# LemonATsu/DANBO-pytorch

Measured on AMD Instinct MI355X. Metric: ray-samples/sec at 512x512x64 samples, higher is better.
Workload: dtype f32 (fp16x2-split MFMA products, fp32 accumulate); 1 GPU; H36M danbo_base network, 512x512 rays x (48 coarse + 16 importance) samples, 1 pose / 1 camera per rank, cylinder near/far, exact in-volume culling; rays=262144, samples_per_ray=64, parallelism=rays-dp1

## Files before the change

### danbo-pytorch_amd/core/_hip.py

```python
import ctypes
import os
import re
from ctypes import c_char_p, c_float, c_int, c_void_p
from types import SimpleNamespace

import torch

_HERE = os.path.dirname(os.path.abspath(__file__))
LIB_PATH = os.environ.get("DANBO_HIP_LIB") or os.path.join(os.path.dirname(_HERE), "libdanbo_hip.so")

P = c_void_p
I = c_int
F = c_float


class HeaderError(ValueError):
    """include/danbo_hip.h left the subset of C that parse_header reads"""


_SCALARS = {"int": c_int, "long": ctypes.c_long, "long long": ctypes.c_longlong, "size_t": ctypes.c_size_t, "float": c_float,
            **{f"{u}int{n}_t": getattr(ctypes, f"c_{u}int{n}") for u in ("", "u") for n in (8, 16, 32, 64)}}
_TAIL = r"((?:\*\s*(?:const\b\s*)?)*)(\w+)\s*(?:\[\s*(\w*)\s*\])?$"
_DECL = re.compile(r"(?:const\s+)?(long\s+long|\w+)\b\s*" + _TAIL)
_MORE = re.compile(_TAIL)
# ... 139 lines not shown

def _header_path():
    env = os.environ.get("DANBO_HIP_HEADER")
    tried = [env] if env else [os.path.join(os.path.dirname(LIB_PATH), "danbo_hip.h"),
                               os.path.join(os.path.dirname(os.path.dirname(_HERE)), "include", "danbo_hip.h")]
    for p in tried:
        if os.path.exists(p):
            return p
    raise RuntimeError("danbo_hip.h not found (the ctypes binding is derived from it): tried " + ", ".join(tried)
                       + "; set DANBO_HIP_HEADER or put the header beside the library")


HEADER_PATH = _header_path()
with open(HEADER_PATH) as _f:
    _functions, _structs, _constants = parse_header(_f.read())
SIGNATURES = {name: argtypes for name, (_, argtypes) in _functions.items()}
RESTYPES = {name: restype for name, (restype, _) in _functions.items()}
STRUCTS = {name: type(name, (ctypes.Structure,), {"_fields_": fields, "__doc__": f"struct {name} of include/danbo_hip.h"})
           for name, fields in _structs.items()}
globals().update(STRUCTS)
C = SimpleNamespace(**_constants)
MAX_ROW_SPANS = C.DANBO_MAX_ROW_SPANS
ANERF_MAX_D = C.DANBO_ANERF_MAX_D

TRAIN_TENSORS = (
    ["graph_net.layers.0.lin.weight", "graph_net.layers.0.adj_w", "graph_net.layers.0.bias", "graph_net.layers.1.lin.weight",
     "graph_net.layers.1.adj_w", "graph_net.layers.1.bias", "graph_net.layers.2.weight", "graph_net.layers.2.bias",
     "graph_net.layers.3.weight", "graph_net.layers.3.bias", "graph_net.axis_scale",
     "prob_linears.layers.0.lin.weight", "prob_linears.layers.0.adj_w", "prob_linears.layers.0.bias", "prob_linears.layers.1.weight",
     "prob_linears.layers.1.bias", "prob_linears.layers.2.weight", "prob_linears.layers.2.bias"]
# ... 6 lines not shown
            "framecodes.codes.weight": C.DANBO_T_CODES}
if len(TRAIN_TENSORS) != N_TRAIN_TENSORS or any(TRAIN_TENSORS.index(k) != i for k, i in _anchors.items()):
    raise HeaderError(f"TRAIN_TENSORS does not line up with enum DanboTrainTensor of {HEADER_PATH}")

_lib = None


def lib():
    global _lib
    if _lib is None:
        if not os.path.exists(LIB_PATH):
            raise RuntimeError(
                f"{LIB_PATH} not found: build it with `make -C danbo-pytorch_amd/csrc` "
                "(or __graft_entry__.build()).  There is no CPU / PyTorch fallback.")
        l = ctypes.CDLL(LIB_PATH)
        for name, argtypes in SIGNATURES.items():
            fn = getattr(l, name)
            fn.argtypes = argtypes
            fn.restype = RESTYPES[name]
        if l.danbo_abi_version() != C.DANBO_ABI_VERSION:
            raise RuntimeError(f"{LIB_PATH} has ABI version {l.danbo_abi_version()}, {HEADER_PATH} declares {C.DANBO_ABI_VERSION}: "
                               "the library is stale, rebuild it with `make -C danbo-pytorch_amd/csrc`")
        _lib = l
    return _lib


def ptr(t):
    return None if t is None else c_void_p(t.data_ptr())


def stream():
    return c_void_p(torch.cuda.current_stream().cuda_stream)


# ... 12 lines not shown
```

### danbo-pytorch_amd/core/hip_ops.py

```python
import ctypes

import torch

from . import _hip
from ._hip import call as _call, ptr as _p, stream as _stream

J = _hip.C.DANBO_J
VOL = _hip.C.DANBO_VOL
FEAT = _hip.C.DANBO_FEAT
RAY_FLAT_VMAX = _hip.C.DANBO_RAY_FLAT_VMAX
H_STRIDE = _hip.C.DANBO_H_STRIDE
MLP_PACKED_FLOATS = _hip.C.DANBO_MLP_PACKED_FLOATS
ASSIGN16_PACKED_BYTES = _hip.C.DANBO_ASSIGN16_PACKED_BYTES
MLP16_PACKED_BYTES = _hip.C.DANBO_MLP16_PACKED_BYTES
ANERF_ENC_FLOATS = _hip.C.DANBO_ANERF_ENC_FLOATS
LINEAR16_ENC_K = _hip.C.DANBO_LINEAR16_ENC_K
TRUNK_PACKED_BYTES = _hip.C.DANBO_TRUNK_PACKED_BYTES
TRUNK_PE_WIDTH = _hip.C.DANBO_TRUNK_PE_WIDTH
VIEW_W = 128


def _f32(t, name):
    if t is None:
        return None
# ... 78 lines not shown


def bone_cull(geo, compact=True, cnt=None):
    bits = torch.empty(geo.M, device=geo.device, dtype=torch.int32)
    lst = None
    if compact:
        lst = torch.empty(geo.M, device=geo.device, dtype=torch.int32)
        if cnt is None:
            cnt = torch.zeros(1, device=geo.device, dtype=torch.int32)
        assert cnt.dtype == torch.int32 and cnt.numel() == 1 and cnt.is_contiguous()
    else:
        cnt = None
    rm = tuple(geo.ray_mask) if geo.ray_mask is not None else (None, None, None)
    flat = rm[3] if len(rm) > 3 else None
    _call("danbo_bone_cull", *geo.head(), _p(rm[0]), _p(rm[1]), _p(rm[2]), _p(flat), _p(bits), _p(lst), _p(cnt), _stream())
    return bits, lst, cnt


def ray_bone_mask(rays_o, rays_d, skts, align, axis_scale, t_lo, t_hi, want_flat=False):
    rays_o, rays_d, skts = _f32(rays_o, "rays_o"), _f32(rays_d, "rays_d"), _f32(skts, "skts")
    t_lo, t_hi = _f32(t_lo, "t_lo").reshape(-1), _f32(t_hi, "t_hi").reshape(-1)
    R, G = rays_o.shape[0], skts.shape[0]
    assert t_lo.shape[0] == R and t_hi.shape[0] == R
    mask = torch.empty(R, device=rays_o.device, dtype=torch.int32)
    flat = torch.empty(R, device=rays_o.device, dtype=torch.int32) if want_flat else None
    _call("danbo_ray_bone_mask", _p(rays_o), _p(rays_d), _p(t_lo), _p(t_hi), R, G, _p(skts), _p(_f32(align, "align")),
          _p(_f32(axis_scale, "axis_scale")), _p(mask), _p(flat), _stream())
    return (mask, t_lo, t_hi, flat) if want_flat else (mask, t_lo, t_hi)


# ... 626 lines not shown
```

### danbo-pytorch_amd/core/render_engine.py

```python
import ctypes

import torch

from . import _hip
from . import hip_ops as ops


class RenderEngine:
    fuse_resample = False

    def _key(self):
        return tuple((k, v.data_ptr(), v._version) for k, v in sorted(self.p.items()))

    def _sampling(self, N_samples, N_importance):
        cfg = self.cfg
        return (N_samples or cfg["N_samples"], N_importance or cfg["N_importance"], cfg["density_scale"],
                ops.density_act(cfg.get("density_act")))

    @staticmethod
    def frame_result(out, out0):
        return dict(rgb_map=out["rgb_map"], disp_map=out["disp_map"], acc_map=out["acc_map"], alpha=out["alpha"],
                    T_i=out["weights"], rgb0=out0["rgb_map"], disp0=out0["disp_map"], acc0=out0["acc_map"],
                    alpha0=out0["alpha"])

# ... 161 lines not shown
        self.refresh()
        return ops.pose_volumes(bones, self.gw, self.cfg["multires_graph"])

    def view_constants(self, rays_d, skts, cam_idx, ray_list=None, ray_count=None):
        self.refresh()
        cfg = self.cfg
        ray_mode = {"world": 0, "root_local": 1}[cfg["ray_tr_type"]]
        normalise = 1 if cfg["view_type"] == "relray" else 0
        return ops.view_consts(rays_d, skts, ray_mode, normalise, cfg["multires_views"], self.framecodes,
                               self.mean_code, cam_idx, self.wrt,
                               self.views_b16 if self.mlp_mode == "f16split" else self.views_b, self.rgb_w,
                               self.rgb_b, self.empty_consts, {16: 1, 32: 2}[self.mlp_form] if self.mlp_mode == "f16split" else 0,
                               self.code_table, ray_list, ray_count)

    def forward_samples(self, rays_o, rays_d, skts, bones, cam_idx=None, z=None, pts=None, dense=False,
                        want_confd=False, volumes=None, view=None, fill=True, ray_mask=None, count=None):
        self.refresh()
        geo = ops.Geometry(rays_o, rays_d, skts, self.align, self.axis_scale, z=z, pts=pts, ray_mask=ray_mask)
        vols = self.volumes(bones) if volumes is None else volumes
        cview, raw_empty = self.view_constants(geo.rays_d, geo.skts, cam_idx) if view is None else view
        S = geo.S
        bits, lst, cnt = ops.bone_cull(geo, compact=not dense, cnt=count)
        if lst is not None and self.mlp_mode == "f16split" and self.group_rows:
            ops.group_rows(bits, lst, cnt)
        if self.mlp_mode == "f16split":
            h, confd = ops.gather_assign_blend16(geo, vols, bits, self.aw, self.assign16, lst, cnt, geo.M, want_confd)
        else:
            h, confd = ops.gather_assign_blend(geo, vols, bits, self.aw, lst, cnt, geo.M, want_confd)
        raw = ops.fill_raw(raw_empty, S) if fill or dense else torch.empty(geo.R, S, 4, device=raw_empty.device)
        if self.profile is not None:
            e0, e1 = torch.cuda.Event(enable_timing=True), torch.cuda.Event(enable_timing=True)
            e0.record()
        self._mlp(h, S, cview, raw, lst, cnt, geo.M)
        if self.profile is not None:
            e1.record()
            self.profile.setdefault("k_pe_mlp", []).append((e0, e1, cnt if cnt is not None else geo.M))
        extras = dict(valid_bits=bits, list=lst, count=cnt, confd_rows=confd, h_rows=h, volumes=vols)
# ... 75 lines not shown
        self.refresh()
        near, far = ops.near_far_cylinder(rays_o, rays_d, cyls, near0, far0, chunk)
        if self.cfg["use_volume_near_far"]:
            ops.near_far_boxes(rays_o, rays_d, skts, self.align, self.axis_scale, near, far)
        return near, far

    def render(self, rays_o, rays_d, skts, bones, cyls, cam_idx=None, N_samples=None, N_importance=None,
               chunk=4096, near_far=None, dense=False, keep=False):
        S, Sf, B, act = self._sampling(N_samples, N_importance)
        self.refresh()
        fused = S <= 64 and Sf <= 64
        lazy = not dense and not keep
        flat_mode = (lazy and (fused or (S <= 256 and Sf <= 64)) and self.skip_flat_rays and self.flat_rays_ok
                     and act[0] == "relu")
        near, far = self.near_far(rays_o, rays_d, cyls, skts, 0.0, 1.0, chunk) if near_far is None else near_far
        z = ops.coarse_samples(near, far, S)
        ray_mask = None if dense else ops.ray_bone_mask(rays_o, rays_d, skts, self.align, self.axis_scale, near, far,
                                                        want_flat=flat_mode)
        counts = torch.zeros(3, device=rays_o.device, dtype=torch.int32)
        flat = None
        vols = self.volumes(bones)
        if flat_mode:
            flat = ops.flat_rays(ray_mask[1], ray_mask[3], S, Sf, want_weights=not fused, cnt=counts[2:3])
            view = self.view_constants(rays_d, skts, cam_idx, flat["ray_list"], flat["ray_count"])
        else:
            view = self.view_constants(rays_d, skts, cam_idx)
        if ray_mask is not None:
            ray_mask = ray_mask[:3]
        raw, ex = self.forward_samples(rays_o, rays_d, skts, bones, cam_idx, z=z, dense=dense, volumes=vols, view=view,
                                       fill=not lazy, ray_mask=ray_mask, count=counts[0:1])
        if fused:
            out0, z_all, z_fine, order = ops.composite_importance(
                raw, z, rays_d, Sf, B, bits=ex["valid_bits"] if lazy else None, raw_empty=view[1] if lazy else None,
                want_weights=keep, flat=flat, act=act)
        else:
            out0 = ops.composite(raw, z, rays_d, B, bits=ex["valid_bits"] if lazy else None, raw_empty=view[1] if lazy else None,
                                 flat=flat, act=act)
            z_all, z_fine, order = ops.importance_samples(z, out0["weights"], Sf, flat=flat)
        raw_f, ex_f = self.forward_samples(rays_o, rays_d, skts, bones, cam_idx, z=z_fine, dense=dense,
                                           volumes=vols, view=view, fill=not lazy,
                                           ray_mask=ray_mask, count=counts[1:2])
        out = ops.composite_merged(raw, raw_f, order, z_all, rays_d, B, bits_a=ex["valid_bits"] if lazy else None,
                                   bits_b=ex_f["valid_bits"] if lazy else None, raw_empty=view[1] if lazy else None,
                                   want_raw=keep, flat=flat, act=act)
        ret = self.frame_result(out, out0)
        if keep:
            ret.update(near=near, far=far, z_coarse=z, raw_coarse=raw, weights_coarse=out0["weights"], z_fine=z_fine,
                       z_sorted=z_all, sorted_idxs=order, raw_fine=raw_f, raw_sorted=out.get("raw_sorted"),
                       count_coarse=ex["count"], count_fine=ex_f["count"], valid_bits=ex["valid_bits"])
        return ret

    def _network_pass(self, rays_o, rays_d, skts, bones, cam_idx, z, bounds, dense, lazy, tag):
        mask = None if dense else ops.ray_bone_mask(rays_o, rays_d, skts, self.align, self.axis_scale, *bounds)
        view = self.view_constants(rays_d, skts, cam_idx)
        raw, ex = self.forward_samples(rays_o, rays_d, skts, bones, cam_idx, z=z, dense=dense, volumes=self.volumes(bones), view=view,
                                       fill=not lazy, ray_mask=mask)
# ... 3 lines not shown
```

### danbo-pytorch_amd/csrc/common.hpp

```cpp
#pragma once
#include <hip/hip_runtime.h>
#include <stdint.h>
#include <algorithm>
#include <atomic>
#include "../../include/danbo_hip.h"
#include "sample_math.hpp"

#define DANBO_CHECK_ARG(cond) do { if (!(cond)) return DANBO_EINVAL; } while (0)
#define DANBO_CHECK_DENSITY_ACT(act, shift) \
    DANBO_CHECK_ARG(((act) == DANBO_DENSITY_RELU || (act) == DANBO_DENSITY_SOFTPLUS) && (shift) - (shift) == 0.f)
#define DANBO_TRY(call) do { const int rc_ = (call); if (rc_ != 0) return rc_; } while (0)
#define DANBO_LAUNCH_RET() do { hipError_t e_ = hipGetLastError(); return e_ == hipSuccess ? 0 : (int)e_; } while (0)

#define DANBO_ENSURE_LDS(func, bytes)                                                                              \
    do {                                                                                                           \
        static std::atomic<unsigned long long> done_{0};                                                           \
        int dev_ = 0;                                                                                              \
        if (hipGetDevice(&dev_) != hipSuccess) return (int)hipGetLastError();                                      \
        const unsigned long long bit_ = 1ull << (dev_ & 63);                                                       \
        if (!(done_.load(std::memory_order_acquire) & bit_)) {                                                     \
            const hipError_t e_ = hipFuncSetAttribute(reinterpret_cast<const void*>(func),                         \
                                                      hipFuncAttributeMaxDynamicSharedMemorySize, (int)(bytes));   \
            if (e_ != hipSuccess) return (int)e_;                                                                  \
            done_.fetch_or(bit_, std::memory_order_release);                                                       \
// ... 183 lines not shown
```

### danbo-pytorch_amd/csrc/k_frame.hip

```cpp
#include "common.hpp"

using namespace danbo;

namespace {
struct FrameBuffers {
    float *near, *far, *cyl_scratch, *z, *vol_scratch, *volumes, *cview, *raw_empty, *h, *raw_a, *raw_b, *z_fine, *z_sorted, *weights0;
    uint32_t *bits_a, *bits_b, *ray_mask, *ray_flat;
    int32_t *list, *count, *order, *ray_list;
};

FrameBuffers carve(Carver& c, int R, int G, int S, int Sf, int chunk, int Wg) {
    FrameBuffers b;
    const size_t M = (size_t)R * S, Mf = (size_t)R * Sf;
    b.near = c.take<float>(R);
    b.far = c.take<float>(R);
    b.cyl_scratch = c.take<float>(8 * (size_t)((R + chunk - 1) / chunk));
    b.z = c.take<float>(M);
    b.vol_scratch = c.take<float>(3 * (size_t)G * 24 * Wg);
    b.volumes = c.take<float>((size_t)G * 24 * 240);
    b.cview = c.take<float>((size_t)R * 128);
    b.raw_empty = c.take<float>((size_t)R * 4);
    b.ray_mask = c.take<uint32_t>(R);
    b.ray_flat = c.take<uint32_t>(R);
    b.ray_list = c.take<int32_t>(R);
// ... 25 lines not shown
    DANBO_CHECK_ARG(m && r && o && workspace && S >= 3 && S <= 256 && Sf >= 1 && Sf <= 64);
    DANBO_CHECK_ARG(r->R >= 1 && r->G >= 1 && r->R % r->G == 0 && r->chunk >= 1);
    DANBO_CHECK_ARG(r->rays_o && r->rays_d && r->skts && r->bones && r->cyls);
    DANBO_CHECK_ARG(o->rgb_map && o->disp_map && o->acc_map && o->alpha && o->weights && o->rgb0 && o->disp0 && o->acc0 && o->alpha0);
    const int R = r->R, G = r->G;
    const bool flat_rays = m->flat_rays_ok != 0 && act == DANBO_DENSITY_RELU;
    DANBO_CHECK_ARG(workspace_bytes >= danbo_render_frame_workspace(R, G, S, Sf, r->chunk, m->graph_width));
    Carver c(workspace);
    const FrameBuffers b = carve(c, R, G, S, Sf, r->chunk, m->graph_width);
    hipStream_t st = (hipStream_t)stream;

    DANBO_TRY(danbo_near_far_cylinder(r->rays_o, r->rays_d, r->cyls, R, G, 0.f, 1.f, r->near_in, r->far_in, r->chunk, b.cyl_scratch,
                                      b.near, b.far, stream));
    if (m->use_volume_near_far)
        DANBO_TRY(danbo_near_far_boxes(r->rays_o, r->rays_d, r->skts, m->align, m->axis_scale, R, G, b.near, b.far, stream));
    DANBO_TRY(danbo_coarse_samples(b.near, b.far, R, S, nullptr, b.z, stream));
    DANBO_TRY(danbo_ray_bone_mask(r->rays_o, r->rays_d, b.near, b.far, R, G, r->skts, m->align, m->axis_scale, b.ray_mask,
                                  flat_rays ? b.ray_flat : nullptr, stream));
    DANBO_TRY(danbo_pose_volumes_fwd(r->bones, G, m->L_graph, m->graph_width, m->g_w0, m->g_adjw0, m->g_b0, m->g_w1, m->g_adjw1, m->g_b1,
                                     m->g_w2, m->g_b2, m->g_w3, m->g_b3, b.vol_scratch, b.volumes, stream));
    zero_words(b.count, 4, nullptr, 0, st);
    auto view_consts = [&](const int32_t* ray_list, const int32_t* ray_count) -> int {
        return danbo_view_consts(r->rays_d, r->skts, R, G, m->ray_mode, m->normalise, m->L_view, m->framecodes, m->n_codes, m->code_size,
                                 m->mean_code, r->cam_idx, m->views_w_ray_t, m->views_b_eff, m->rgb_w, m->rgb_b, m->empty_consts, 2,
                                 m->code_table, ray_list, ray_count, b.cview, b.raw_empty, stream);
    };
    const int32_t *ray_list = nullptr, *ray_count = nullptr;
    if (flat_rays) {
        DANBO_TRY(danbo_flat_rays(b.near, b.ray_flat, R, S, Sf, o->rgb0, o->disp0, o->acc0, b.weights0, o->alpha0, b.z_fine, o->rgb_map,
                                  o->disp_map, o->acc_map, o->weights, o->alpha, b.ray_list, b.count + 3, 3, stream));
        ray_list = b.ray_list;
        ray_count = b.count + 3;
    }
    DANBO_TRY(view_consts(ray_list, ray_count));
    auto cull = [&](const float* zz, int s, uint32_t* bits, int32_t* count) -> int {
        DANBO_TRY(danbo_bone_cull(r->rays_o, r->rays_d, zz, nullptr, R, s, G, r->skts, m->align, m->axis_scale, b.ray_mask, b.near, b.far,
                                  nullptr, bits, b.list, count, stream));
        return 0;
    };
    auto network = [&](const float* zz, int s, uint32_t* bits, int32_t* count, float* raw) -> int {
        DANBO_TRY(danbo_gather_assign_blend16_fwd(r->rays_o, r->rays_d, zz, nullptr, R, s, G, r->skts, m->align, m->axis_scale, b.volumes,
                                                  bits, b.list, count, R * s, m->assign16, m->a_b0, m->a_b1, m->a_w2, m->a_b2, b.h,
                                                  nullptr, reinterpret_cast<uint32_t*>(b.count + 2), stream));
        return danbo_pe_mlp32_fwd(b.h, b.list, count, R * s, s, m->mlp16, m->pts_b, m->alpha_w, m->alpha_b, b.cview, m->rgb_w,
                                  m->rgb_b, raw, nullptr, stream);
    };
    DANBO_TRY(cull(b.z, S, b.bits_a, b.count));
    DANBO_TRY(network(b.z, S, b.bits_a, b.count, b.raw_a));
    if (S <= 64) {
        DANBO_TRY(danbo_composite_importance_pdf_fwd_act(b.raw_a, b.raw_empty, b.bits_a, b.z, r->rays_d, R, S, Sf, m->density_scale, nullptr,
                                                         nullptr, 0, o->rgb0, o->disp0, o->acc0, nullptr, o->alpha0, b.z_fine, b.z_sorted,
                                                         b.order, ray_list, ray_count, act, shift, stream));
    } else {
        DANBO_TRY(danbo_composite_rays_fwd_act(b.raw_a, b.raw_empty, b.bits_a, b.z, r->rays_d, R, S, m->density_scale, nullptr, o->rgb0,
                                               o->disp0, o->acc0, b.weights0, o->alpha0, ray_list, ray_count, act, shift, stream));
        DANBO_TRY(danbo_importance_samples_rays(b.z, b.weights0, R, S, Sf, nullptr, b.z_fine, b.z_sorted, b.order, ray_list, ray_count,
                                                stream));
    }
    DANBO_TRY(cull(b.z_fine, Sf, b.bits_b, b.count + 1));
    DANBO_TRY(network(b.z_fine, Sf, b.bits_b, b.count + 1, b.raw_b));
    return danbo_composite_merged_fwd_act(b.raw_a, b.raw_b, b.raw_empty, b.bits_a, b.bits_b, b.order, b.z_sorted, r->rays_d, R, S, Sf,
                                          m->density_scale, nullptr, o->rgb_map, o->disp_map, o->acc_map, o->weights, o->alpha, nullptr,
                                          ray_list, ray_count, act, shift, stream);
}

extern "C" int danbo_render_frame(const DanboModel* m, const DanboRays* r, int S, int Sf, const DanboFrameOut* o, void* workspace,
                                  size_t workspace_bytes, void* stream) {
    return render_frame_impl(m, r, S, Sf, o, workspace, workspace_bytes, DANBO_DENSITY_RELU, 0.f, stream);
}

extern "C" int danbo_render_frame_act(const DanboModel* m, const DanboRays* r, int S, int Sf, const DanboFrameOut* o, void* workspace,
                                      size_t workspace_bytes, int act, float shift, void* stream) {
    DANBO_CHECK_DENSITY_ACT(act, shift);
    return render_frame_impl(m, r, S, Sf, o, workspace, workspace_bytes, act, act == DANBO_DENSITY_SOFTPLUS ? shift : 0.f, stream);
// ... 2 lines not shown
```

### danbo-pytorch_amd/csrc/k_sample.hip

```cpp
#include "common.hpp"

namespace danbo {

__global__ __launch_bounds__(256) DANBO_NO_PK_F32 void k_cylinder_pass1(const float* __restrict__ rays_o,
                                                        const float* __restrict__ rays_d,
                                                        const float* __restrict__ cyl, int R, int G,
                                                        float near0, float far0,
                                                        const float* __restrict__ near_in,
                                                        const float* __restrict__ far_in, int chunk,
                                                        double* __restrict__ acc,
                                                        float* __restrict__ near_out,
                                                        float* __restrict__ far_out) {
    const int rays_per_pose = R / G;
    for (int r0 = blockIdx.x * blockDim.x; r0 < R; r0 += gridDim.x * blockDim.x) {
        const int r = r0 + threadIdx.x;
        const bool act = r < R;
        const int rc = act ? r : R - 1;
        const int g = min(rc / rays_per_pose, G - 1);
        float o[3] = {rays_o[3 * rc], rays_o[3 * rc + 1], rays_o[3 * rc + 2]};
        float d[3] = {rays_d[3 * rc], rays_d[3 * rc + 1], rays_d[3 * rc + 2]};
        float c[3] = {cyl[5 * g], cyl[5 * g + 1], cyl[5 * g + 2]};
        float nr, fr;
        const bool hit = cylinder_bounds(o, d, c, near_in ? near_in[rc] : near0, far_in ? far_in[rc] : far0, &nr, &fr) && act;
        if (act) {
// ... 307 lines not shown
            const float* m0 = POSES_IN_LDS ? s_skt + (size_t)(g - g0) * J * 16 : skts + (size_t)g * J * 16;
            float msum = 0.f;
            for (int a = 0; a < 3; ++a)
                for (int k = 0; k < 3; ++k) msum = add_rn(msum, fabsf(m0[4 * a + k]));
            const float vin = mul_rn(dn, fmaxf(1.0f, msum));
            const bool fin = zl <= zh && sub_rn(span, span) == 0.f && sub_rn(tail, tail) == 0.f && vin <= RAY_FLAT_VMAX;
            ray_flat[r] = (bits == 0u && fin) ? 1u : 0u;
        }
    }
}

constexpr int CULL_BLOCK = 256;
constexpr int CULL_SPT = 4;
constexpr int CULL_MAX_RAYS = 130;

__global__ __launch_bounds__(CULL_BLOCK) void k_bone_cull(const float* __restrict__ rays_o,
                                                          const float* __restrict__ rays_d,
                                                          const float* __restrict__ z,
                                                          const float* __restrict__ pts, int R, int S, int G,
                                                          const float* __restrict__ skts,
                                                          const float* __restrict__ align,
                                                          const float* __restrict__ axis_scale, int np_lds,
                                                          const uint32_t* __restrict__ ray_mask,
                                                          const float* __restrict__ t_lo, const float* __restrict__ t_hi,
                                                          uint32_t* __restrict__ ray_flat,
                                                          uint32_t* __restrict__ valid_bits,
                                                          int32_t* __restrict__ list, int32_t* __restrict__ count) {
    extern __shared__ __attribute__((aligned(16))) float smem[];
    float* s_align = smem;
    float* s_scale = smem + J * 16;
// ... 1 lines not shown
    __shared__ float s_zlo[CULL_MAX_RAYS], s_zhi[CULL_MAX_RAYS];
    __shared__ uint32_t s_mask[CULL_MAX_RAYS];

    const long M = (long)R * S;
    const long spp = (long)(R / G) * S;
    const long base = (long)blockIdx.x * (CULL_BLOCK * CULL_SPT);
    const long last = min(base + CULL_BLOCK * CULL_SPT, M) - 1;
    const int g0 = (int)min(base / spp, (long)G - 1);
    const int g1 = (int)min(last / spp, (long)G - 1);

    const int lane = threadIdx.x & 63;
    const int r_first = (int)(base / S), r_last = (int)(last / S);
    const int off0 = (int)(base - (long)r_first * S);
    const int rays_per_pose = R / G;
    const float inv_S = 1.0f / (float)S;
    auto ray_of = [&](int li) {
        int q = (int)((float)li * inv_S);
        q -= (q * S > li) ? 1 : 0;
        q += ((q + 1) * S <= li) ? 1 : 0;
        return q;
    };
    auto pose_of = [&](int r) { return G == 1 ? 0 : min(r / rays_per_pose, G - 1); };
    const int nrays = r_last - r_first + 1;
    const bool prefilter = pts == nullptr && ray_mask == nullptr && nrays <= CULL_MAX_RAYS;
    float zreg[CULL_SPT];
    if (pts == nullptr) {
#pragma unroll
        for (int k = 0; k < CULL_SPT; ++k) zreg[k] = z[min(base + k * CULL_BLOCK + threadIdx.x, M - 1)];
    }
    uint32_t pre[CULL_SPT];
    if (ray_mask != nullptr) {
        bool any = false;
#pragma unroll
        for (int k = 0; k < CULL_SPT; ++k) {
            pre[k] = 0u;
            if (base + k * CULL_BLOCK + threadIdx.x < M) {
                const int r = r_first + ray_of(off0 + k * CULL_BLOCK + threadIdx.x);
                const float lo = t_lo[r], hi = t_hi[r];
                const float slack = 5e-5f * fmaxf(fabsf(lo), fabsf(hi));
                const bool inside = zreg[k] >= lo - slack && zreg[k] <= hi + slack;
                pre[k] = inside ? ray_mask[r] : (1u << J) - 1u;
                if (!inside && ray_flat != nullptr) ray_flat[r] = 0u;
            }
            any = any || pre[k] != 0u;
        }
        if (!__syncthreads_or(any ? 1 : 0)) {
#pragma unroll
            for (int k = 0; k < CULL_SPT; ++k)
                if (base + k * CULL_BLOCK + threadIdx.x < M) valid_bits[base + k * CULL_BLOCK + threadIdx.x] = 0u;
            return;
        }
    }
    for (int i = threadIdx.x; i < J * 16; i += CULL_BLOCK) s_align[i] = align[i];
    for (int i = threadIdx.x; i < J * 4; i += CULL_BLOCK) s_scale[i] = (i & 3) < 3 ? fabsf(axis_scale[(i >> 2) * 3 + (i & 3)]) : 0.f;
    const int npose = g1 - g0 + 1;
    for (int i = threadIdx.x; i < npose * J * 16; i += CULL_BLOCK) s_skt[i] = skts[(size_t)g0 * J * 16 + i];
// ... 50 lines not shown
            const float da[3] = {rays_d[3 * ra], rays_d[3 * ra + 1], rays_d[3 * ra + 2]};
            const float ob[3] = {rays_o[3 * rb], rays_o[3 * rb + 1], rays_o[3 * rb + 2]};
            const float db[3] = {rays_d[3 * rb], rays_d[3 * rb + 1], rays_d[3 * rb + 2]};
            sample_point(oa, da, ma < M ? zreg[2 * pr] : z[M - 1], pa);
            sample_point(ob, db, mb < M ? zreg[2 * pr + 1] : z[M - 1], pb);
        }
        const int ga = pose_of(ra), gb = pose_of(rb);
        uint32_t ba = 0, bb = 0;
        uint32_t need = (1u << J) - 1u;
        if (ray_mask != nullptr) {
            need = wave_or(pre[2 * pr] | pre[2 * pr + 1]);
        } else if (prefilter) {
            uint32_t mine = s_mask[ra - r_first] | s_mask[rb - r_first];
            need = wave_or(mine);
        }
        if (__builtin_amdgcn_readfirstlane((int)__all(ga == gb))) {
            const v2f px = {pa[0], pb[0]}, py = {pa[1], pb[1]}, pz = {pa[2], pb[2]};
            const float* sk = s_skt + (ga - g0) * J * 16;
            while (need) {
                const int j = __builtin_ctz(need);
                need &= need - 1u;
                v2f l[3], t[3];
                affine_pk(sk + 16 * j, px, py, pz, l);
                affine_pk(s_align + 16 * j, l[0], l[1], l[2], t);
                const float* sc = s_scale + 4 * j;
                const bool ina = !(fabsf(t[0].x) > sc[0] || fabsf(t[1].x) > sc[1] || fabsf(t[2].x) > sc[2]);
                const bool inb = !(fabsf(t[0].y) > sc[0] || fabsf(t[1].y) > sc[1] || fabsf(t[2].y) > sc[2]);
                ba |= (ina ? 1u : 0u) << j;
                bb |= (inb ? 1u : 0u) << j;
            }
        } else {
            const float* ska = s_skt + (ga - g0) * J * 16;
            const float* skb = s_skt + (gb - g0) * J * 16;
            for (int j = 0; j < J; ++j) {
                float pt[3];
                bone_local(ska + 16 * j, s_align + 16 * j, pa, pt);
                ba |= (in_volume(pt, s_scale + 4 * j) ? 1u : 0u) << j;
                bone_local(skb + 16 * j, s_align + 16 * j, pb, pt);
                bb |= (in_volume(pt, s_scale + 4 * j) ? 1u : 0u) << j;
            }
        }
        bits4[2 * pr] = ma < M ? ba : 0u;
        bits4[2 * pr + 1] = mb < M ? bb : 0u;
        if (ma < M) valid_bits[ma] = ba;
        if (mb < M) valid_bits[mb] = bb;
    }
    if (list != nullptr) {
        __shared__ int s_cnt[CULL_SPT * (CULL_BLOCK / 64)];
        __shared__ int s_base;
        const int wave = threadIdx.x >> 6;
        unsigned long long ball[CULL_SPT];
#pragma unroll
        for (int it = 0; it < CULL_SPT; ++it) {
            ball[it] = __ballot(bits4[it] != 0);
            if (lane == 0) s_cnt[it * (CULL_BLOCK / 64) + wave] = __popcll(ball[it]);
        }
        __syncthreads();
        if (threadIdx.x == 0) {
            int run = 0;
            for (int i = 0; i < CULL_SPT * (CULL_BLOCK / 64); ++i) { const int c = s_cnt[i]; s_cnt[i] = run; run += c; }
            s_base = run > 0 ? atomicAdd(count, run) : 0;
        }
        __syncthreads();
#pragma unroll
        for (int it = 0; it < CULL_SPT; ++it) {
            if (bits4[it] != 0) {
                const long m = base + it * CULL_BLOCK + threadIdx.x;
                list[s_base + s_cnt[it * (CULL_BLOCK / 64) + wave] + __popcll(ball[it] & ((1ull << lane) - 1ull))] = (int32_t)m;
            }
        }
    }
}

constexpr int GATHER_TS = 16;
constexpr int GATHER_BLOCK = GATHER_TS * J;

__global__ __launch_bounds__(GATHER_BLOCK) void k_bone_gather(const float* __restrict__ rays_o,
                                                              const float* __restrict__ rays_d,
                                                              const float* __restrict__ z,
                                                              const float* __restrict__ pts, int R, int S, int G,
                                                              const float* __restrict__ skts,
                                                              const float* __restrict__ align,
                                                              const float* __restrict__ axis_scale,
                                                              const float* __restrict__ volumes,
                                                              const int32_t* __restrict__ list,
                                                              const int32_t* __restrict__ count, int n_cap,
// ... 616 lines not shown
    DANBO_CHECK_ARG(ray_mask == nullptr || (z != nullptr && t_lo != nullptr && t_hi != nullptr));
    DANBO_CHECK_ARG(ray_flat == nullptr || ray_mask != nullptr);
    const long M = (long)R * S;
    const long spp = (long)(R / G) * S;
    const int per_block = CULL_BLOCK * CULL_SPT;
    long np = per_block / spp + 2;
    if (np > G) np = G;
    const size_t lds = sizeof(float) * (J * 16 + J * 4 + np * J * 16);
    DANBO_CHECK_ARG(lds <= 64 * 1024);
    const int grid = ceil_div(M, per_block);
    hipLaunchKernelGGL(k_bone_cull, dim3(grid), dim3(CULL_BLOCK), lds, (hipStream_t)stream, rays_o, rays_d, z, pts, R, S,
                       G, skts, align, axis_scale, (int)np, ray_mask, t_lo, t_hi, ray_flat, valid_bits, list, count);
    DANBO_LAUNCH_RET();
}

extern "C" int danbo_ray_bone_mask(const float* rays_o, const float* rays_d, const float* t_lo, const float* t_hi, int R, int G,
                                    const float* skts, const float* align, const float* axis_scale, uint32_t* ray_mask,
                                    uint32_t* ray_flat, void* stream) {
    DANBO_CHECK_ARG(rays_o && rays_d && t_lo && t_hi && skts && align && axis_scale && ray_mask);
    DANBO_CHECK_ARG(R > 0 && G > 0 && R % G == 0);
    const long np = 256 / (R / G) + 2 < G ? 256 / (R / G) + 2 : G;
    const bool in_lds = np <= 8;
    const size_t lds = sizeof(float) * (J * 16 + J * 4 + (in_lds ? np * J * 16 : 0));
    if (in_lds)
        hipLaunchKernelGGL(k_ray_bone_mask<true>, dim3(ceil_div(R, 256)), dim3(256), lds, (hipStream_t)stream, rays_o, rays_d, t_lo, t_hi,
                           skts, align, axis_scale, R, G, ray_mask, ray_flat);
    else
        hipLaunchKernelGGL(k_ray_bone_mask<false>, dim3(ceil_div(R, 256)), dim3(256), lds, (hipStream_t)stream, rays_o, rays_d, t_lo,
                           t_hi, skts, align, axis_scale, R, G, ray_mask, ray_flat);
    DANBO_LAUNCH_RET();
// ... 240 lines not shown
```

Measured before the change: 4.092 billion ray-samples/s.

## Cull only listed non-flat rays and generate coarse z inside the cull kernel

Adds a new bone-cull kernel that iterates over the compacted list of rays that hit any bone volume, instead of over all R*S samples. In the flat-ray mode it also computes the coarse sample depths inside the cull kernel and skips the separate coarse_samples launch. The goal is to cut cull work and memory traffic for rays that miss the body, and to remove one kernel launch and one z pass. In exchange, valid_bits and z are no longer written for culled rays, so downstream code must rely on the ray list, and the launch grid is sized for all R rays, with blocks past the live count returning early.

```diff
diff --git a/danbo-pytorch_amd/core/_hip.py b/danbo-pytorch_amd/core/_hip.py
--- a/danbo-pytorch_amd/core/_hip.py
+++ b/danbo-pytorch_amd/core/_hip.py
@@ -177,6 +177,17 @@
 HEADER_PATH = _header_path()
 with open(HEADER_PATH) as _f:
     _functions, _structs, _constants = parse_header(_f.read())
+INTERNAL_HEADER_PATH = next((p for p in (os.path.join(os.path.dirname(LIB_PATH), "danbo_internal.h"),
+                                         os.path.join(os.path.dirname(_HERE), "csrc", "danbo_internal.h")) if os.path.exists(p)), None)
+if INTERNAL_HEADER_PATH is None:
+    raise RuntimeError("danbo_internal.h not found beside the library or under csrc/ (the binding of the internal entry points is "
+                       "derived from it)")
+with open(INTERNAL_HEADER_PATH) as _f:
+    _internal = parse_header(_f.read())[0]
+if set(_internal) & set(_functions):
+    raise HeaderError(f"{INTERNAL_HEADER_PATH} declares entry points of {HEADER_PATH} again: {sorted(set(_internal) & set(_functions))}")
+INTERNAL_SIGNATURES = {name: argtypes for name, (_, argtypes) in _internal.items()}
+INTERNAL_RESTYPES = {name: restype for name, (restype, _) in _internal.items()}
 SIGNATURES = {name: argtypes for name, (_, argtypes) in _functions.items()}
 RESTYPES = {name: restype for name, (restype, _) in _functions.items()}
 STRUCTS = {name: type(name, (ctypes.Structure,), {"_fields_": fields, "__doc__": f"struct {name} of include/danbo_hip.h"})
@@ -213,10 +224,10 @@
                 f"{LIB_PATH} not found: build it with `make -C danbo-pytorch_amd/csrc` "
                 "(or __graft_entry__.build()).  There is no CPU / PyTorch fallback.")
         l = ctypes.CDLL(LIB_PATH)
-        for name, argtypes in SIGNATURES.items():
+        for name, argtypes in {**SIGNATURES, **INTERNAL_SIGNATURES}.items():
             fn = getattr(l, name)
             fn.argtypes = argtypes
-            fn.restype = RESTYPES[name]
+            fn.restype = RESTYPES.get(name) or INTERNAL_RESTYPES[name]
         if l.danbo_abi_version() != C.DANBO_ABI_VERSION:
             raise RuntimeError(f"{LIB_PATH} has ABI version {l.danbo_abi_version()}, {HEADER_PATH} declares {C.DANBO_ABI_VERSION}: "
                                "the library is stale, rebuild it with `make -C danbo-pytorch_amd/csrc`")
diff --git a/danbo-pytorch_amd/core/hip_ops.py b/danbo-pytorch_amd/core/hip_ops.py
--- a/danbo-pytorch_amd/core/hip_ops.py
+++ b/danbo-pytorch_amd/core/hip_ops.py
@@ -116,6 +116,17 @@
     rm = tuple(geo.ray_mask) if geo.ray_mask is not None else (None, None, None)
     flat = rm[3] if len(rm) > 3 else None
     _call("danbo_bone_cull", *geo.head(), _p(rm[0]), _p(rm[1]), _p(rm[2]), _p(flat), _p(bits), _p(lst), _p(cnt), _stream())
+    return bits, lst, cnt
+
+
+def bone_cull_rays(geo, flat, cnt, make_z=False):
+    assert geo.z is not None and geo.ray_mask is not None and cnt.dtype == torch.int32 and cnt.numel() == 1 and cnt.is_contiguous()
+    bits = torch.empty(geo.M, device=geo.device, dtype=torch.int32)
+    lst = torch.empty(geo.M, device=geo.device, dtype=torch.int32)
+    rm = geo.ray_mask
+    _call("danbo_bone_cull_rays", _p(geo.rays_o), _p(geo.rays_d), _p(geo.z), int(bool(make_z)), geo.R, geo.S, geo.G, _p(geo.skts),
+          _p(geo.align), _p(geo.axis_scale), _p(rm[0]), _p(rm[1]), _p(rm[2]), _p(flat["ray_list"]), _p(flat["ray_count"]), _p(bits),
+          _p(lst), _p(cnt), _stream())
     return bits, lst, cnt
 
 
diff --git a/danbo-pytorch_amd/core/render_engine.py b/danbo-pytorch_amd/core/render_engine.py
--- a/danbo-pytorch_amd/core/render_engine.py
+++ b/danbo-pytorch_amd/core/render_engine.py
@@ -199,13 +199,18 @@
                                self.code_table, ray_list, ray_count)
 
     def forward_samples(self, rays_o, rays_d, skts, bones, cam_idx=None, z=None, pts=None, dense=False,
-                        want_confd=False, volumes=None, view=None, fill=True, ray_mask=None, count=None):
+                        want_confd=False, volumes=None, view=None, fill=True, ray_mask=None, count=None, rays=None,
+                        make_z=False):
         self.refresh()
         geo = ops.Geometry(rays_o, rays_d, skts, self.align, self.axis_scale, z=z, pts=pts, ray_mask=ray_mask)
         vols = self.volumes(bones) if volumes is None else volumes
         cview, raw_empty = self.view_constants(geo.rays_d, geo.skts, cam_idx) if view is None else view
         S = geo.S
-        bits, lst, cnt = ops.bone_cull(geo, compact=not dense, cnt=count)
+        if rays is not None:
+            assert not dense
+            bits, lst, cnt = ops.bone_cull_rays(geo, rays, count, make_z)
+        else:
+            bits, lst, cnt = ops.bone_cull(geo, compact=not dense, cnt=count)
         if lst is not None and self.mlp_mode == "f16split" and self.group_rows:
             ops.group_rows(bits, lst, cnt)
         if self.mlp_mode == "f16split":
@@ -311,7 +316,7 @@
         flat_mode = (lazy and (fused or (S <= 256 and Sf <= 64)) and self.skip_flat_rays and self.flat_rays_ok
                      and act[0] == "relu")
         near, far = self.near_far(rays_o, rays_d, cyls, skts, 0.0, 1.0, chunk) if near_far is None else near_far
-        z = ops.coarse_samples(near, far, S)
+        z = torch.empty(near.shape[0], S, device=near.device, dtype=torch.float32) if flat_mode else ops.coarse_samples(near, far, S)
         ray_mask = None if dense else ops.ray_bone_mask(rays_o, rays_d, skts, self.align, self.axis_scale, near, far,
                                                         want_flat=flat_mode)
         counts = torch.zeros(3, device=rays_o.device, dtype=torch.int32)
@@ -325,7 +330,7 @@
         if ray_mask is not None:
             ray_mask = ray_mask[:3]
         raw, ex = self.forward_samples(rays_o, rays_d, skts, bones, cam_idx, z=z, dense=dense, volumes=vols, view=view,
-                                       fill=not lazy, ray_mask=ray_mask, count=counts[0:1])
+                                       fill=not lazy, ray_mask=ray_mask, count=counts[0:1], rays=flat, make_z=flat_mode)
         if fused:
             out0, z_all, z_fine, order = ops.composite_importance(
                 raw, z, rays_d, Sf, B, bits=ex["valid_bits"] if lazy else None, raw_empty=view[1] if lazy else None,
@@ -336,7 +341,7 @@
             z_all, z_fine, order = ops.importance_samples(z, out0["weights"], Sf, flat=flat)
         raw_f, ex_f = self.forward_samples(rays_o, rays_d, skts, bones, cam_idx, z=z_fine, dense=dense,
                                            volumes=vols, view=view, fill=not lazy,
-                                           ray_mask=ray_mask, count=counts[1:2])
+                                           ray_mask=ray_mask, count=counts[1:2], rays=flat)
         out = ops.composite_merged(raw, raw_f, order, z_all, rays_d, B, bits_a=ex["valid_bits"] if lazy else None,
                                    bits_b=ex_f["valid_bits"] if lazy else None, raw_empty=view[1] if lazy else None,
                                    want_raw=keep, flat=flat, act=act)
diff --git a/danbo-pytorch_amd/csrc/common.hpp b/danbo-pytorch_amd/csrc/common.hpp
--- a/danbo-pytorch_amd/csrc/common.hpp
+++ b/danbo-pytorch_amd/csrc/common.hpp
@@ -4,6 +4,7 @@
 #include <algorithm>
 #include <atomic>
 #include "../../include/danbo_hip.h"
+#include "danbo_internal.h"
 #include "sample_math.hpp"
 
 #define DANBO_CHECK_ARG(cond) do { if (!(cond)) return DANBO_EINVAL; } while (0)
diff --git a/danbo-pytorch_amd/csrc/danbo_internal.h b/danbo-pytorch_amd/csrc/danbo_internal.h
--- /dev/null
+++ b/danbo-pytorch_amd/csrc/danbo_internal.h
@@ -0,0 +1,21 @@
+#ifndef DANBO_INTERNAL_H
+#define DANBO_INTERNAL_H
+
+#include <stddef.h>
+#include <stdint.h>
+
+#ifdef __cplusplus
+extern "C" {
+#endif
+
+int danbo_bone_cull_rays(const float* rays_o, const float* rays_d, float* z ,
+                         int make_z, int R, int S, int G, const float* skts , const float* align ,
+                         const float* axis_scale , const uint32_t* ray_mask , const float* t_lo ,
+                         const float* t_hi , const int32_t* ray_list , const int32_t* ray_count ,
+                         uint32_t* valid_bits , int32_t* list , int32_t* count , void* stream);
+
+#ifdef __cplusplus
+}
+#endif
+
+#endif
diff --git a/danbo-pytorch_amd/csrc/k_frame.hip b/danbo-pytorch_amd/csrc/k_frame.hip
--- a/danbo-pytorch_amd/csrc/k_frame.hip
+++ b/danbo-pytorch_amd/csrc/k_frame.hip
@@ -63,7 +63,7 @@
                                       b.near, b.far, stream));
     if (m->use_volume_near_far)
         DANBO_TRY(danbo_near_far_boxes(r->rays_o, r->rays_d, r->skts, m->align, m->axis_scale, R, G, b.near, b.far, stream));
-    DANBO_TRY(danbo_coarse_samples(b.near, b.far, R, S, nullptr, b.z, stream));
+    if (!flat_rays) DANBO_TRY(danbo_coarse_samples(b.near, b.far, R, S, nullptr, b.z, stream));
     DANBO_TRY(danbo_ray_bone_mask(r->rays_o, r->rays_d, b.near, b.far, R, G, r->skts, m->align, m->axis_scale, b.ray_mask,
                                   flat_rays ? b.ray_flat : nullptr, stream));
     DANBO_TRY(danbo_pose_volumes_fwd(r->bones, G, m->L_graph, m->graph_width, m->g_w0, m->g_adjw0, m->g_b0, m->g_w1, m->g_adjw1, m->g_b1,
@@ -82,9 +82,14 @@
         ray_count = b.count + 3;
     }
     DANBO_TRY(view_consts(ray_list, ray_count));
-    auto cull = [&](const float* zz, int s, uint32_t* bits, int32_t* count) -> int {
-        DANBO_TRY(danbo_bone_cull(r->rays_o, r->rays_d, zz, nullptr, R, s, G, r->skts, m->align, m->axis_scale, b.ray_mask, b.near, b.far,
-                                  nullptr, bits, b.list, count, stream));
+    auto cull = [&](float* zz, int s, uint32_t* bits, int32_t* count, bool coarse) -> int {
+        if (ray_list) {
+            DANBO_TRY(danbo_bone_cull_rays(r->rays_o, r->rays_d, zz, coarse ? 1 : 0, R, s, G, r->skts, m->align, m->axis_scale, b.ray_mask,
+                                           b.near, b.far, ray_list, ray_count, bits, b.list, count, stream));
+        } else {
+            DANBO_TRY(danbo_bone_cull(r->rays_o, r->rays_d, zz, nullptr, R, s, G, r->skts, m->align, m->axis_scale, b.ray_mask, b.near,
+                                      b.far, nullptr, bits, b.list, count, stream));
+        }
         return 0;
     };
     auto network = [&](const float* zz, int s, uint32_t* bits, int32_t* count, float* raw) -> int {
@@ -94,7 +99,7 @@
         return danbo_pe_mlp32_fwd(b.h, b.list, count, R * s, s, m->mlp16, m->pts_b, m->alpha_w, m->alpha_b, b.cview, m->rgb_w,
                                   m->rgb_b, raw, nullptr, stream);
     };
-    DANBO_TRY(cull(b.z, S, b.bits_a, b.count));
+    DANBO_TRY(cull(b.z, S, b.bits_a, b.count, true));
     DANBO_TRY(network(b.z, S, b.bits_a, b.count, b.raw_a));
     if (S <= 64) {
         DANBO_TRY(danbo_composite_importance_pdf_fwd_act(b.raw_a, b.raw_empty, b.bits_a, b.z, r->rays_d, R, S, Sf, m->density_scale, nullptr,
@@ -106,7 +111,7 @@
         DANBO_TRY(danbo_importance_samples_rays(b.z, b.weights0, R, S, Sf, nullptr, b.z_fine, b.z_sorted, b.order, ray_list, ray_count,
                                                 stream));
     }
-    DANBO_TRY(cull(b.z_fine, Sf, b.bits_b, b.count + 1));
+    DANBO_TRY(cull(b.z_fine, Sf, b.bits_b, b.count + 1, false));
     DANBO_TRY(network(b.z_fine, Sf, b.bits_b, b.count + 1, b.raw_b));
     return danbo_composite_merged_fwd_act(b.raw_a, b.raw_b, b.raw_empty, b.bits_a, b.bits_b, b.order, b.z_sorted, r->rays_d, R, S, Sf,
                                           m->density_scale, nullptr, o->rgb_map, o->disp_map, o->acc_map, o->weights, o->alpha, nullptr,
diff --git a/danbo-pytorch_amd/csrc/k_sample.hip b/danbo-pytorch_amd/csrc/k_sample.hip
--- a/danbo-pytorch_amd/csrc/k_sample.hip
+++ b/danbo-pytorch_amd/csrc/k_sample.hip
@@ -345,6 +345,48 @@
 constexpr int CULL_SPT = 4;
 constexpr int CULL_MAX_RAYS = 130;
 
+__device__ __forceinline__ int cull_div(int li, int S, float inv_S ) {
+    int q = (int)((float)li * inv_S);
+    q -= (q * S > li) ? 1 : 0;
+    q += ((q + 1) * S <= li) ? 1 : 0;
+    return q;
+}
+__device__ __forceinline__ uint32_t cull_candidates(float z, float lo, float hi, const uint32_t* mask, bool* inside) {
+    const float slack = 5e-5f * fmaxf(fabsf(lo), fabsf(hi));
+    *inside = z >= lo - slack && z <= hi + slack;
+    return *inside ? *mask : (1u << J) - 1u;
+}
+__device__ __forceinline__ void cull_test_pair(const float* ska, const float* skb, bool same_pose, const float* s_align,
+                                               const float* s_scale, const float* pa, const float* pb, uint32_t need,
+                                               uint32_t* ba_out, uint32_t* bb_out) {
+    uint32_t ba = 0, bb = 0;
+    if (__builtin_amdgcn_readfirstlane((int)__all(same_pose))) {
+        const v2f px = {pa[0], pb[0]}, py = {pa[1], pb[1]}, pz = {pa[2], pb[2]};
+        while (need) {
+            const int j = __builtin_ctz(need);
+            need &= need - 1u;
+            v2f l[3], t[3];
+            affine_pk(ska + 16 * j, px, py, pz, l);
+            affine_pk(s_align + 16 * j, l[0], l[1], l[2], t);
+            const float* sc = s_scale + 4 * j;
+            const bool ina = !(fabsf(t[0].x) > sc[0] || fabsf(t[1].x) > sc[1] || fabsf(t[2].x) > sc[2]);
+            const bool inb = !(fabsf(t[0].y) > sc[0] || fabsf(t[1].y) > sc[1] || fabsf(t[2].y) > sc[2]);
+            ba |= (ina ? 1u : 0u) << j;
+            bb |= (inb ? 1u : 0u) << j;
+        }
+    } else {
+        for (int j = 0; j < J; ++j) {
+            float pt[3];
+            bone_local(ska + 16 * j, s_align + 16 * j, pa, pt);
+            ba |= (in_volume(pt, s_scale + 4 * j) ? 1u : 0u) << j;
+            bone_local(skb + 16 * j, s_align + 16 * j, pb, pt);
+            bb |= (in_volume(pt, s_scale + 4 * j) ? 1u : 0u) << j;
+        }
+    }
+    *ba_out = ba;
+    *bb_out = bb;
+}
+
 __global__ __launch_bounds__(CULL_BLOCK) void k_bone_cull(const float* __restrict__ rays_o,
                                                           const float* __restrict__ rays_d,
                                                           const float* __restrict__ z,
@@ -376,12 +418,7 @@
     const int off0 = (int)(base - (long)r_first * S);
     const int rays_per_pose = R / G;
     const float inv_S = 1.0f / (float)S;
-    auto ray_of = [&](int li) {
-        int q = (int)((float)li * inv_S);
-        q -= (q * S > li) ? 1 : 0;
-        q += ((q + 1) * S <= li) ? 1 : 0;
-        return q;
-    };
+    auto ray_of = [&](int li) { return cull_div(li, S, inv_S); };
     auto pose_of = [&](int r) { return G == 1 ? 0 : min(r / rays_per_pose, G - 1); };
     const int nrays = r_last - r_first + 1;
     const bool prefilter = pts == nullptr && ray_mask == nullptr && nrays <= CULL_MAX_RAYS;
@@ -398,10 +435,8 @@
             pre[k] = 0u;
             if (base + k * CULL_BLOCK + threadIdx.x < M) {
                 const int r = r_first + ray_of(off0 + k * CULL_BLOCK + threadIdx.x);
-                const float lo = t_lo[r], hi = t_hi[r];
-                const float slack = 5e-5f * fmaxf(fabsf(lo), fabsf(hi));
-                const bool inside = zreg[k] >= lo - slack && zreg[k] <= hi + slack;
-                pre[k] = inside ? ray_mask[r] : (1u << J) - 1u;
+                bool inside;
+                pre[k] = cull_candidates(zreg[k], t_lo[r], t_hi[r], ray_mask + r, &inside);
                 if (!inside && ray_flat != nullptr) ray_flat[r] = 0u;
             }
             any = any || pre[k] != 0u;
@@ -482,32 +517,7 @@
             uint32_t mine = s_mask[ra - r_first] | s_mask[rb - r_first];
             need = wave_or(mine);
         }
-        if (__builtin_amdgcn_readfirstlane((int)__all(ga == gb))) {
-            const v2f px = {pa[0], pb[0]}, py = {pa[1], pb[1]}, pz = {pa[2], pb[2]};
-            const float* sk = s_skt + (ga - g0) * J * 16;
-            while (need) {
-                const int j = __builtin_ctz(need);
-                need &= need - 1u;
-                v2f l[3], t[3];
-                affine_pk(sk + 16 * j, px, py, pz, l);
-                affine_pk(s_align + 16 * j, l[0], l[1], l[2], t);
-                const float* sc = s_scale + 4 * j;
-                const bool ina = !(fabsf(t[0].x) > sc[0] || fabsf(t[1].x) > sc[1] || fabsf(t[2].x) > sc[2]);
-                const bool inb = !(fabsf(t[0].y) > sc[0] || fabsf(t[1].y) > sc[1] || fabsf(t[2].y) > sc[2]);
-                ba |= (ina ? 1u : 0u) << j;
-                bb |= (inb ? 1u : 0u) << j;
-            }
-        } else {
-            const float* ska = s_skt + (ga - g0) * J * 16;
-            const float* skb = s_skt + (gb - g0) * J * 16;
-            for (int j = 0; j < J; ++j) {
-                float pt[3];
-                bone_local(ska + 16 * j, s_align + 16 * j, pa, pt);
-                ba |= (in_volume(pt, s_scale + 4 * j) ? 1u : 0u) << j;
-                bone_local(skb + 16 * j, s_align + 16 * j, pb, pt);
-                bb |= (in_volume(pt, s_scale + 4 * j) ? 1u : 0u) << j;
-            }
-        }
+        cull_test_pair(s_skt + (ga - g0) * J * 16, s_skt + (gb - g0) * J * 16, ga == gb, s_align, s_scale, pa, pb, need, &ba, &bb);
         bits4[2 * pr] = ma < M ? ba : 0u;
         bits4[2 * pr + 1] = mb < M ? bb : 0u;
         if (ma < M) valid_bits[ma] = ba;
@@ -538,6 +548,126 @@
             }
         }
     }
+}
+
+constexpr int CULL_RAYS_W = 4;
+constexpr int CULL_RAYS_ITEMS = CULL_RAYS_W * CULL_BLOCK * CULL_SPT;
+constexpr int CULL_RAYS_POSES_LDS = 8;
+static inline int cull_rays_per_wg(int S) { return CULL_RAYS_ITEMS / S; }
+
+template <bool MAKE_Z, bool POSES_IN_LDS>
+__global__ __launch_bounds__(CULL_BLOCK) void k_bone_cull_rays(const float* __restrict__ rays_o, const float* __restrict__ rays_d,
+                                                               float* __restrict__ z, int R, int S, int G, int rays_per_wg,
+                                                               const float* __restrict__ skts, const float* __restrict__ align,
+                                                               const float* __restrict__ axis_scale,
+                                                               const uint32_t* __restrict__ ray_mask, const float* __restrict__ t_lo,
+                                                               const float* __restrict__ t_hi, const int32_t* __restrict__ ray_list,
+                                                               const int32_t* __restrict__ ray_count,
+                                                               uint32_t* __restrict__ valid_bits, int32_t* __restrict__ list,
+                                                               int32_t* __restrict__ count) {
+    extern __shared__ __attribute__((aligned(16))) float smem[];
+    float* s_align = smem;
+    float* s_scale = smem + J * 16;
+    float* s_skt = smem + J * 16 + J * 4;
+    constexpr int WIN = CULL_BLOCK * CULL_SPT, WAVES = CULL_BLOCK / 64, NCNT = CULL_RAYS_W * CULL_SPT * WAVES;
+    __shared__ int s_cnt[NCNT];
+
+    const int n_rays = min(max(*ray_count, 0), R);
+    const int slot0 = blockIdx.x * rays_per_wg;
+    if (slot0 >= n_rays) return;
+    const int n_items = min(rays_per_wg, n_rays - slot0) * S;
+    for (int i = threadIdx.x; i < J * 16; i += CULL_BLOCK) s_align[i] = align[i];
+    for (int i = threadIdx.x; i < J * 4; i += CULL_BLOCK) s_scale[i] = (i & 3) < 3 ? fabsf(axis_scale[(i >> 2) * 3 + (i & 3)]) : 0.f;
+    if (POSES_IN_LDS)
+        for (int i = threadIdx.x; i < G * J * 16; i += CULL_BLOCK) s_skt[i] = skts[i];
+    __syncthreads();
+
+    const int lane = threadIdx.x & 63, wave = threadIdx.x >> 6;
+    const int rays_per_pose = R / G;
+    const float inv_S = 1.0f / (float)S;
+    int mm[CULL_RAYS_W][CULL_SPT];
+#pragma unroll
+    for (int w = 0; w < CULL_RAYS_W; ++w) {
+#pragma unroll
+        for (int k = 0; k < CULL_SPT; ++k) mm[w][k] = -1;
+        if (w * WIN >= n_items) continue;
+#pragma unroll
+        for (int pr = 0; pr < CULL_SPT / 2; ++pr) {
+            const int ia = w * WIN + (2 * pr) * CULL_BLOCK + threadIdx.x, ib = ia + CULL_BLOCK;
+            const int lia = min(ia, n_items - 1), lib = min(ib, n_items - 1);
+            const int qa = cull_div(lia, S, inv_S), qb = cull_div(lib, S, inv_S);
+            const int sa = lia - qa * S, sb = lib - qb * S;
+            const int ra = (int)min((unsigned)ray_list[slot0 + qa], (unsigned)(R - 1));
+            const int rb = (int)min((unsigned)ray_list[slot0 + qb], (unsigned)(R - 1));
+            const int ma = ra * S + sa, mb = rb * S + sb;
+            const float oa[3] = {rays_o[3 * ra], rays_o[3 * ra + 1], rays_o[3 * ra + 2]};
+            const float da[3] = {rays_d[3 * ra], rays_d[3 * ra + 1], rays_d[3 * ra + 2]};
+            const float ob[3] = {rays_o[3 * rb], rays_o[3 * rb + 1], rays_o[3 * rb + 2]};
+            const float db[3] = {rays_d[3 * rb], rays_d[3 * rb + 1], rays_d[3 * rb + 2]};
+            const float loa = t_lo[ra], hia = t_hi[ra], lob = t_lo[rb], hib = t_hi[rb];
+            const float za = MAKE_Z ? coarse_z(loa, hia, sa, S) : z[ma];
+            const float zb = MAKE_Z ? coarse_z(lob, hib, sb, S) : z[mb];
+            bool inside;
+            const uint32_t prea = cull_candidates(za, loa, hia, ray_mask + ra, &inside);
+            const uint32_t preb = cull_candidates(zb, lob, hib, ray_mask + rb, &inside);
+            float pa[3], pb[3];
+            sample_point(oa, da, za, pa);
+            sample_point(ob, db, zb, pb);
+            const int ga = G == 1 ? 0 : min(ra / rays_per_pose, G - 1), gb = G == 1 ? 0 : min(rb / rays_per_pose, G - 1);
+            const float* sk = POSES_IN_LDS ? s_skt : skts;
+            uint32_t ba, bb;
+            cull_test_pair(sk + (size_t)ga * J * 16, sk + (size_t)gb * J * 16, ga == gb, s_align, s_scale, pa, pb,
+                           wave_or(prea | preb), &ba, &bb);
+            if (ia < n_items) {
+                valid_bits[ma] = ba;
+                if (MAKE_Z) z[ma] = za;
+                if (ba != 0u) mm[w][2 * pr] = ma;
+            }
+            if (ib < n_items) {
+                valid_bits[mb] = bb;
+                if (MAKE_Z) z[mb] = zb;
+                if (bb != 0u) mm[w][2 * pr + 1] = mb;
+            }
+        }
+    }
+#pragma unroll
+    for (int w = 0; w < CULL_RAYS_W; ++w)
+#pragma unroll
+        for (int it = 0; it < CULL_SPT; ++it) {
+            const unsigned long long b = __ballot(mm[w][it] >= 0);
+            if (lane == 0) s_cnt[(w * CULL_SPT + it) * WAVES + wave] = (int)__popcll(b);
+        }
+    __syncthreads();
+    if (wave == 0) {
+        constexpr int E = (NCNT + 63) / 64;
+        int c[E], sum = 0;
+#pragma unroll
+        for (int e = 0; e < E; ++e) { c[e] = lane * E + e < NCNT ? s_cnt[lane * E + e] : 0; sum += c[e]; }
+        int incl = sum;
+#pragma unroll
+        for (int off = 1; off < 64; off <<= 1) {
+            const int t = __shfl_up(incl, off, 64);
+            if (lane >= off) incl += t;
+        }
+        const int total = __shfl(incl, 63, 64);
+        int start = 0;
+        if (lane == 0 && total > 0) start = atomicAdd(count, total);
+        int run = __shfl(start, 0, 64) + incl - sum;
+#pragma unroll
+        for (int e = 0; e < E; ++e) {
+            if (lane * E + e < NCNT) s_cnt[lane * E + e] = run;
+            run += c[e];
+        }
+    }
+    __syncthreads();
+#pragma unroll
+    for (int w = 0; w < CULL_RAYS_W; ++w)
+#pragma unroll
+        for (int it = 0; it < CULL_SPT; ++it) {
+            const unsigned long long b = __ballot(mm[w][it] >= 0);
+            if (mm[w][it] >= 0)
+                list[s_cnt[(w * CULL_SPT + it) * WAVES + wave] + (int)__popcll(b & ((1ull << lane) - 1ull))] = mm[w][it];
+        }
 }
 
 constexpr int GATHER_TS = 16;
@@ -1184,6 +1314,26 @@
     DANBO_LAUNCH_RET();
 }
 
+extern "C" int danbo_bone_cull_rays(const float* rays_o, const float* rays_d, float* z, int make_z, int R, int S, int G,
+                                     const float* skts, const float* align, const float* axis_scale, const uint32_t* ray_mask,
+                                     const float* t_lo, const float* t_hi, const int32_t* ray_list, const int32_t* ray_count,
+                                     uint32_t* valid_bits, int32_t* list, int32_t* count, void* stream) {
+    DANBO_CHECK_ARG(rays_o && rays_d && z && skts && align && axis_scale && ray_mask && t_lo && t_hi && ray_list && ray_count);
+    DANBO_CHECK_ARG(valid_bits && list && count && (make_z == 0 || make_z == 1));
+    DANBO_CHECK_ARG(R > 0 && S > 0 && S <= CULL_BLOCK * CULL_SPT && G > 0 && R % G == 0 && (long)R * S <= 0x7fffffffL);
+    const bool in_lds = G <= CULL_RAYS_POSES_LDS;
+    const size_t lds = sizeof(float) * (J * 16 + J * 4 + (in_lds ? G * J * 16 : 0));
+    const int per_wg = cull_rays_per_wg(S);
+    const dim3 grid(ceil_div(R, per_wg)), block(CULL_BLOCK);
+    auto launch = [&](auto kernel) {
+        hipLaunchKernelGGL(kernel, grid, block, lds, (hipStream_t)stream, rays_o, rays_d, z, R, S, G, per_wg, skts, align, axis_scale,
+                           ray_mask, t_lo, t_hi, ray_list, ray_count, valid_bits, list, count);
+    };
+    if (make_z) in_lds ? launch(k_bone_cull_rays<true, true>) : launch(k_bone_cull_rays<true, false>);
+    else in_lds ? launch(k_bone_cull_rays<false, true>) : launch(k_bone_cull_rays<false, false>);
+    DANBO_LAUNCH_RET();
+}
+
 extern "C" int danbo_ray_bone_mask(const float* rays_o, const float* rays_d, const float* t_lo, const float* t_hi, int R, int G,
                                     const float* skts, const float* align, const float* axis_scale, uint32_t* ray_mask,
                                     uint32_t* ray_flat, void* stream) {
```

Measured after the change: 4.130 billion ray-samples/s, median of 6. About the same (+0.9%).
